# mako443/Text2Pos-CVPR2022

Measured on AMD Instinct MI355X. Metric: cells+queries encoded/sec and top-k retrieval QPS, 256-pt cells, 12k-cell DB, higher is better.
Workload: dtype f16x3 (fp32 operands split hi+lo into fp16, 3 f16 MFMAs, fp32 accumulate; fp32-class error) for the encoders / f64 MFMA for the ranking

## Files before the change

### text2pos-cvpr2022_amd/csrc/sa_rows.hip

```cpp
#ifndef T2P_RABL
#define T2P_RABL 0
#endif
#include "t2p_common.h"

namespace t2p {
namespace {

typedef __attribute__((address_space(3))) void lds_void;
typedef const __attribute__((address_space(1))) void gl_void;

__device__ __forceinline__ constexpr int rows_load_slot(int s, int c) {
    if (s == 0) return c == 0 || c == 4 ? -1 : 10 + (c < 4 ? c - 1 : c - 2);
    if (s == 1) return c == 1 ? 16 : (c == 3 ? 17 : -1);
    if (s == 4) return (c & 1) ? 18 + (c >> 1) : -1;
    if (s == 5) return (c & 1) ? 22 + (c >> 1) : -1;
    return -1;
}
#ifndef T2P_WA_HI_STEPS
#define T2P_WA_HI_STEPS 3
#endif
constexpr int WA_HI_STEPS = T2P_WA_HI_STEPS;
__device__ __forceinline__ constexpr bool w_in_agpr(bool lo_plane, int s) { return lo_plane || s < WA_HI_STEPS; }
__device__ __forceinline__ void mfma_w(f32x16& c, const half8& a, const half8& w, bool agpr, bool zero) {
    if (zero) {
        if (agpr) asm volatile("v_mfma_f32_32x32x16_f16 %0, %1, %2, 0" : "=a"(c) : "v"(a), "a"(w));
        else asm volatile("v_mfma_f32_32x32x16_f16 %0, %1, %2, 0" : "=a"(c) : "v"(a), "v"(w));
    } else {
        if (agpr) asm volatile("v_mfma_f32_32x32x16_f16 %0, %1, %2, %0" : "+a"(c) : "v"(a), "a"(w));
        else asm volatile("v_mfma_f32_32x32x16_f16 %0, %1, %2, %0" : "+a"(c) : "v"(a), "v"(w));
    }
}
#define SB() __builtin_amdgcn_sched_barrier(0)
#if T2P_RABL & 2
#define DS_MAX_STR "; no atomic %0 %1 %2"
#else
#define DS_MAX_STR "ds_max_f32 %0, %1 offset:%2"
#endif

constexpr int kSubR = 1024;

template <int K, int N, int NC, int NW>
struct RowsCfg {
    static constexpr int NT = 64 * NW;
    static constexpr int ND = 2 * NC;
    static constexpr int S16 = K / 16, NTW = N / 32;
    static constexpr int MAXR = NC * 33;
    static constexpr int ROWS_CHUNKS = (MAXR * 2 + 1023) / 1024;
    static constexpr int ROWS_BUF = ROWS_CHUNKS * 1024;
    static constexpr int BT_STRIDE = K * 4 + 16;
    static constexpr int CPOS_BUF = 3 * NC * 4;
    static constexpr int ACC_OFF = 0;
    static constexpr int XROW = kSaTailCode;
    static constexpr int BT_OFF = ACC_OFF + (NC + 1) * N * 4;
    static constexpr int ROWS_OFF = BT_OFF + NC * BT_STRIDE;
    static constexpr int CPOS_OFF = ROWS_OFF + 3 * ROWS_BUF;
    static constexpr int NR_OFF = CPOS_OFF + 2 * CPOS_BUF;
    static constexpr int SB_OFF = NR_OFF + kSubR * 2;
    static constexpr int DSTL_OFF = SB_OFF + kSubR * 4;
    static constexpr size_t lds_bytes() { return (size_t)(DSTL_OFF + NW * 64 + 1023) / 1024 * 1024; }
    static_assert(K % 32 == 0 && N % 32 == 0 && NC % 64 == 0 && (NC * N / 4) % NT == 0, "shape");
    static_assert(K == 128, "rows_load_slot schedules the loads of eight MFMA steps per tile");
    static_assert(XROW == NC && (NC & (NC - 1)) == 0 && XROW * N * 4 <= 0xFFFF && XROW < 128, "shared tail slot");
};

__device__ __forceinline__ void wait_all_vm() { asm volatile("s_waitcnt vmcnt(0)" ::: "memory"); }

struct TileRef {
    int gi, r0, n;
};

template <int K, int N, int NC, int NW>
__global__ __launch_bounds__(64 * NW, 1) void k_sa_rows(SaParams p) {
    using C = RowsCfg<K, N, NC, NW>;
    extern __shared__ __attribute__((aligned(16))) char lds[];
    int* acc_lds = (int*)(lds + C::ACC_OFF);
    uint16_t* nr = (uint16_t*)(lds + C::NR_OFF);
    int* sbase = (int*)(lds + C::SB_OFF);

    const int tid = threadIdx.x, lane = tid & 63;
    const int wave = __builtin_amdgcn_readfirstlane(tid >> 6);
    const int h = lane >> 5, rr = lane & 31;
    const uint32_t dstl_addr = (uint32_t)(C::DSTL_OFF + wave * 64);

    half8 w_hi[C::NTW][C::S16], w_lo[C::NTW][C::S16];
    {
        const uint4* wp = (const uint4*)p.W_x3;
        constexpr int PLANE_U4 = (N / 32) * C::S16 * 64;
#pragma unroll
        for (int nt = 0; nt < C::NTW; nt++)
#pragma unroll
            for (int s = 0; s < C::S16; s++) {
                const int kb = 16 * s + 8 * h;
                const int half_ = kb / (K / 2), step_ = (kb % (K / 2)) / 8;
                const int idx = (((nt * C::S16 + step_) * 2 + half_) * 32) + rr;
                w_hi[nt][s] = __builtin_bit_cast(half8, wp[idx]);
                w_lo[nt][s] = __builtin_bit_cast(half8, wp[PLANE_U4 + idx]);
                if (w_in_agpr(false, s)) asm volatile("" : "=a"(w_hi[nt][s]) : "0"(w_hi[nt][s]));
                asm volatile("" : "=a"(w_lo[nt][s]) : "0"(w_lo[nt][s]));
            }
    }
    f32x4 bias4;
    {
        const int c4 = tid % (N / 4);
        bias4 = *(const f32x4*)(p.bias + c4 * 4);
    }
    constexpr int QPR = K / 4;
    constexpr int CGS = C::NT / QPR;
    constexpr int CPT = NC / CGS;
    static_assert(C::NT % QPR == 0 && NC % CGS == 0, "centroid table build");
    const int cq = tid % QPR, cg = tid / QPR;
    const f32x4 wq0 = *(const f32x4*)(p.wp + cq * 4), wq1 = *(const f32x4*)(p.wp + K + cq * 4),
                wq2 = *(const f32x4*)(p.wp + 2 * K + cq * 4);

    for (int i = tid; i < (NC + 1) * N; i += C::NT) acc_lds[i] = (int)0xFF800000;
    int gtop = 0;

    const int g_begin = p.bounds_ws[blockIdx.x], g_end = p.bounds_ws[blockIdx.x + 1];

    auto dma16 = [&](const void* base, uint32_t voff, uint32_t lds_off) {
        __builtin_amdgcn_global_load_lds((gl_void*)((const char*)base + voff), (lds_void*)(lds + lds_off), 16, 0, 0);
    };
    auto dma_rows = [&](int g) {
        const char* src = (const char*)(p.rows + (int64_t)g * C::MAXR);
        const uint32_t dst = (uint32_t)(C::ROWS_OFF + (g % 3) * C::ROWS_BUF);
#pragma unroll
        for (int c = 0; c < C::ROWS_CHUNKS; c++) {
            if (c % NW != wave) continue;
            uint32_t off = (uint32_t)(c * 1024 + lane * 16);
            if (off + 16 > (uint32_t)(C::MAXR * 2)) off = 0;
            dma16(src, off, dst + c * 1024);
        }
    };
    auto dma_cpos = [&](int g) {
        if (wave != (NW > 1 ? 1 : 0)) return;
        const uint32_t dst = (uint32_t)(C::CPOS_OFF + (g & 1) * C::CPOS_BUF);
#pragma unroll
        for (int e = 0; e < 3; e++)
#pragma unroll
            for (int b = 0; b < NC / 64; b++) {
                const float* src = p.out + ((int64_t)g * NC + b * 64 + lane) * (int64_t)p.ldo + N + e;
                __builtin_amdgcn_global_load_lds((gl_void*)src, (lds_void*)(lds + dst + (e * NC + b * 64) * 4), 4, 0, 0);
            }
    };

    for (int ga = g_begin; ga < g_end; ga += kSubR) {
        const int cnt = (g_end - ga) < kSubR ? (g_end - ga) : kSubR;
        wait_all_vm();
        __syncthreads();
        for (int i = tid; i < cnt; i += C::NT) {
            const int g = ga + i;
            nr[i] = p.n_rows[g];
            const int first = p.first[g];
            sbase[i] = first * C::ND + (g - first) * NC;
        }
        dma_rows(ga);
        if (cnt > 1) dma_rows(ga + 1);
        dma_cpos(ga);
        wait_all_vm();
        __syncthreads();

        auto rows_of = [&](int gi) { return __builtin_amdgcn_readfirstlane((int)nr[gi]); };
        auto tile_meta = [&](int gi, int r0, int n) -> uint32_t {
            int idx = r0 + rr;
            idx = idx < n ? idx : n - 1;
            const uint16_t* rows_l = (const uint16_t*)(lds + C::ROWS_OFF + ((ga + gi) % 3) * C::ROWS_BUF);
            return (uint32_t)rows_l[idx];
        };
        auto row_byte = [&](int gi, uint32_t sb0, uint32_t m) -> uint32_t {
            const uint32_t src = m & 0xFFu, d = m >> 8;
            const uint32_t g = (uint32_t)(ga + gi);
            const uint32_t srow = (d & 0x80u) ? (sb0 + src) : (g * (uint32_t)C::ND + src);
            return srow * (uint32_t)(K * 4);
        };
        constexpr int AHEAD = 5;
        const uint32_t hoff = (uint32_t)(h * 32);
        auto load_half = [&](uint32_t roff, int s_, int j, f32x4 (&x)[2]) {
            if constexpr (!(T2P_RABL & 1)) x[j] = *(const f32x4*)((const char*)p.A + (size_t)roff + (size_t)(s_ * 64 + j * 16));
        };
        auto load_step = [&](uint32_t roff, int s_, f32x4 (&x)[2]) {
            load_half(roff, s_, 0, x);
            load_half(roff, s_, 1, x);
        };

        auto flush = [&](int g, int t0) {
            float* o = p.out + (int64_t)g * NC * (int64_t)p.ldo;
            int top = gtop;
            static_assert(C::NT % (N / 4) == 0, "a thread keeps its column quad over the drain");
            if (t0 < NC) {
                f32x4* const ax = (f32x4*)(acc_lds + C::XROW * N + (tid % (N / 4)) * 4);
                const f32x4 xq = *ax;
#pragma unroll 1
                for (int c = tid / (N / 4); c < NC; c += C::NT / (N / 4)) {
                    if (c < t0) continue;
                    f32x4* a = (f32x4*)(acc_lds + c * N + (tid % (N / 4)) * 4);
                    f32x4 r = *a;
#pragma unroll
                    for (int e = 0; e < 4; e++) r[e] = fmaxf(r[e], xq[e]);
                    *a = r;
                }
                lds_barrier();
                typedef int i32x4 __attribute__((ext_vector_type(4)));
                if (tid < N / 4) *(i32x4*)ax = i32x4{(int)0xFF800000, (int)0xFF800000, (int)0xFF800000, (int)0xFF800000};
            }
#pragma unroll
            for (int k = 0; k < NC * N / 4 / C::NT; k++) {
                const int i = tid + k * C::NT;
                const int c = i / (N / 4), c4 = i % (N / 4);
                typedef int i32x4 __attribute__((ext_vector_type(4)));
                f32x4* a = (f32x4*)(acc_lds + c * N + c4 * 4);
                const f32x4 raw = *a;
                f32x4 v;
#pragma unroll
                for (int e = 0; e < 4; e++) {
                    const float r = fmaxf(raw[e] + bias4[e], 0.f);
                    const int bits = __float_as_int(r);
                    top = bits > top ? bits : top;
                    v[e] = r * p.out_scale;
                }
                *(f32x4*)(o + c * (int64_t)p.ldo + c4 * 4) = v;
                *(i32x4*)a = i32x4{(int)0xFF800000, (int)0xFF800000, (int)0xFF800000, (int)0xFF800000};
            }
            gtop = top;
        };
        auto build_b = [&](int g) {
            const float* cp = (const float*)(lds + C::CPOS_OFF + (g & 1) * C::CPOS_BUF);
#pragma unroll
            for (int i = 0; i < CPT; i++) {
                const int c = cg + CGS * i;
                const float px = cp[c], py = cp[NC + c], pz = cp[2 * NC + c];
                f32x4 v;
#pragma unroll
                for (int e = 0; e < 4; e++) {
                    float a = px * wq0[e];
                    a = fmaf(py, wq1[e], a);
                    a = fmaf(pz, wq2[e], a);
                    v[e] = a;
                }
                *(f32x4*)(lds + C::BT_OFF + c * C::BT_STRIDE + cq * 16) = v;
            }
        };

        build_b(ga);
        if (cnt > 2) dma_rows(ga + 2);
        if (cnt > 1) dma_cpos(ga + 1);
        lds_barrier();

        bool cur_fetched = false;
        uint32_t m_cur = 0;
        uint32_t roff_cur = 0;
        f32x4 xw[C::S16][2];
#pragma unroll
        for (int s0 = 0; s0 < C::S16; s0++) xw[s0][0] = xw[s0][1] = f32x4{0.f, 0.f, 0.f, 0.f};

        for (int gi = 0; gi < cnt; gi++) {
            const int n_g = rows_of(gi), n_g1 = gi + 1 < cnt ? rows_of(gi + 1) : 0;
            const uint32_t sb_g = (uint32_t)__builtin_amdgcn_readfirstlane(sbase[gi]);
            const uint32_t sb_g1 = gi + 1 < cnt ? (uint32_t)__builtin_amdgcn_readfirstlane(sbase[gi + 1]) : 0u;
            int t0;
            {
                static_assert(NC == 64, "one lane per centroid");
                const uint32_t* cp = (const uint32_t*)(lds + C::CPOS_OFF + ((ga + gi) & 1) * C::CPOS_BUF);
                const bool same = lane > 0 && cp[lane] == cp[0] && cp[NC + lane] == cp[NC] && cp[2 * NC + lane] == cp[2 * NC];
                const unsigned long long tm = __ballot(same);
                t0 = tm ? (int)__builtin_ctzll(tm) : NC;
            }
            int r0 = wave * 32;
            bool have = r0 < n_g;
            const bool did_tile = have;
            half8 a_hi, a_lo;
            f32x16 acc[C::NTW];
            bool pend = false;
            uint2 fourp[4] = {};
            auto read_step = [&](int s, uint32_t brow_, f32x4 (&x)[2], f32x4 (&b)[2]) {
#pragma unroll
                for (int j = 0; j < 2; j++) {
                    x[j] = xw[s][j];
                    b[j] = *(const f32x4*)(lds + brow_ + s * 64 + j * 16);
                }
            };
            auto prep_a = [&](int pr, const f32x4 (&x)[2], const f32x4 (&b)[2], float (&v)[2]) {
                const int j = pr >> 1, e0 = (pr & 1) * 2;
                v[0] = fmaxf(x[j][e0] - b[j][e0], 0.f);
                v[1] = fmaxf(x[j][e0 + 1] - b[j][e0 + 1], 0.f);
            };
            auto prep_b = [&](const float (&v)[2], uint32_t& wh, uint32_t& wl) {
                const fp16x2 hh = cvt_pk_f16(v[0], v[1]);
                wh = __builtin_bit_cast(uint32_t, hh);
                wl = split_lo_pk(hh, v[0], v[1]);
            };
            typedef uint32_t u32x4 __attribute__((ext_vector_type(4)));
            auto row_addr = [&](const uint2 (&f4)[4], int e) -> uint32_t {
                const uint32_t pair = (e & 2) ? f4[e >> 2].y : f4[e >> 2].x;
                return (uint32_t)(C::ACC_OFF + rr * 4) + ((e & 1) ? (pair >> 16) : (pair & 0xFFFFu));
            };

            if (have) {
                if (!cur_fetched) {
                    m_cur = tile_meta(gi, r0, n_g);
                    roff_cur = row_byte(gi, sb_g, m_cur) + hoff;
#pragma unroll
                    for (int s0 = 0; s0 < AHEAD; s0++) load_step(roff_cur, s0, xw[s0]);
                }
                {
                    f32x4 x[2], b[2];
                    read_step(0, (uint32_t)C::BT_OFF + ((m_cur >> 8) & (uint32_t)(NC - 1)) * (uint32_t)C::BT_STRIDE + (uint32_t)(h * 32), x, b);
                    uint32_t nh[4], nl[4];
#pragma unroll
                    for (int pr = 0; pr < 4; pr++) {
                        float v[2];
                        prep_a(pr, x, b, v);
                        prep_b(v, nh[pr], nl[pr]);
                    }
                    a_hi = __builtin_bit_cast(half8, u32x4{nh[0], nh[1], nh[2], nh[3]});
                    a_lo = __builtin_bit_cast(half8, u32x4{nl[0], nl[1], nl[2], nl[3]});
                }
            }
            while (have) {
                const bool chain = r0 + NW * 32 < n_g;
                const bool nxt_ok = chain || (gi + 1 < cnt && wave * 32 < n_g1);
                const int gi_n = chain ? gi : (nxt_ok ? gi + 1 : gi);
                const int r0_n = chain ? r0 + NW * 32 : (nxt_ok ? wave * 32 : r0);
                const int n_n = (chain || !nxt_ok) ? n_g : n_g1;
                const uint32_t sb_n = (chain || !nxt_ok) ? sb_g : sb_g1;
                uint32_t m_nxt = tile_meta(gi_n, r0_n, n_n);
                uint32_t roff_n = roff_cur;
                const uint32_t dl = (m_cur >> 8) & 127u;
                const uint32_t brow = (uint32_t)C::BT_OFF + (dl & (uint32_t)(NC - 1)) * (uint32_t)C::BT_STRIDE + (uint32_t)(h * 32);
                asm volatile("ds_write_b16 %0, %1" ::"v"(dstl_addr + (uint32_t)(rr * 2)), "v"(dl * (uint32_t)(N * 4)) : "memory");
                uint2 four[4];

                uint32_t brow_n = 0;

#pragma unroll
                for (int s = 0; s < C::S16 - 1; s++) {
                    f32x4 x[2], b[2];
                    read_step(s + 1, brow, x, b);
                    if (s == C::S16 - 2) {
                        const uint32_t a4 = dstl_addr + (uint32_t)(h * 8);
                        asm volatile("ds_read_b64 %0, %4\n\tds_read_b64 %1, %4 offset:16\n\tds_read_b64 %2, %4 offset:32\n\t"
                                     "ds_read_b64 %3, %4 offset:48"
                                     : "=&v"(four[0]), "=&v"(four[1]), "=&v"(four[2]), "=&v"(four[3]) : "v"(a4) : "memory");
                    }
                    SB();
                    if (s == 0) {
#pragma unroll
                        for (int nt = 0; nt < C::NTW - 1; nt++) mfma_w(acc[nt], a_hi, w_hi[nt][0], w_in_agpr(false, 0), true);
                        if (pend) {
#pragma unroll
                            for (int e = 0; e < 16; e++)
                                asm volatile(DS_MAX_STR ::"v"(row_addr(fourp, e)), "a"(acc[C::NTW - 1][e]), "n"((C::NTW - 1) * 128) : "memory");
                        }
                        mfma_w(acc[C::NTW - 1], a_hi, w_hi[C::NTW - 1][0], w_in_agpr(false, 0), true);
                    } else {
#pragma unroll
                        for (int nt = 0; nt < C::NTW; nt++) mfma_w(acc[nt], a_hi, w_hi[nt][s], w_in_agpr(false, s), false);
                    }
                    SB();
                    uint32_t nh[4], nl[4];
                    float v[2];
                    uint32_t rowbyte_n = 0;
#pragma unroll
                    for (int c = 0; c < 8; c++) {
                        if ((c & 1) == 0) prep_a(c >> 1, x, b, v);
                        else prep_b(v, nh[c >> 1], nl[c >> 1]);
                        if (s == 0) {
                            if (c == 2) rowbyte_n = row_byte(gi_n, sb_n, m_nxt);
                            if (c == 4) roff_n = rowbyte_n + hoff;
                            if (c == 6) brow_n = (uint32_t)C::BT_OFF + ((m_nxt >> 8) & (uint32_t)(NC - 1)) * (uint32_t)C::BT_STRIDE + (uint32_t)(h * 32);
                        }
                        {
                            const int ld = rows_load_slot(s, c);
                            if (ld >= 0) load_half(ld < 2 * C::S16 ? roff_cur : roff_n, (ld >> 1) % C::S16, ld & 1, xw[(ld >> 1) % C::S16]);
                        }
                        if (c < 4) mfma_w(acc[c], a_hi, w_lo[c][s], w_in_agpr(true, s), false);
                        else mfma_w(acc[c - 4], a_lo, w_hi[c - 4][s], w_in_agpr(false, s), false);
                        SB();
                    }
                    a_hi = __builtin_bit_cast(half8, u32x4{nh[0], nh[1], nh[2], nh[3]});
                    a_lo = __builtin_bit_cast(half8, u32x4{nl[0], nl[1], nl[2], nl[3]});
                }
                {
                    constexpr int s = C::S16 - 1;
                    f32x4 x[2], b[2];
                    if (chain) read_step(0, brow_n, x, b);
                    asm volatile("s_waitcnt lgkmcnt(0)\n\ts_nop 1" : "+v"(four[0]), "+v"(four[1]), "+v"(four[2]), "+v"(four[3])::"memory");
                    SB();
                    uint32_t ad[16];
                    uint32_t nh[4], nl[4];
                    float v[2];
#pragma unroll
                    for (int i = 0; i < 3 * C::NTW; i++) {
                        const int nt = i / 3, k = i % 3;
                        if (k == 0) mfma_w(acc[nt], a_hi, w_hi[nt][s], w_in_agpr(false, s), false);
                        else if (k == 1) mfma_w(acc[nt], a_hi, w_lo[nt][s], w_in_agpr(true, s), false);
                        else mfma_w(acc[nt], a_lo, w_hi[nt][s], w_in_agpr(false, s), false);
                        if (i < 4) {
#pragma unroll
                            for (int e = 4 * i; e < 4 * i + 4; e++) ad[e] = row_addr(four, e);
                        }
                        if (chain && i < 8) {
                            if ((i & 1) == 0) prep_a(i >> 1, x, b, v);
                            else prep_b(v, nh[i >> 1], nl[i >> 1]);
                        }
                        if (i >= 4 && ((i - 4) % 3) < 2 && (i - 4) / 3 < C::NTW - 1) {
                            const int nb = (i - 4) / 3, e0 = ((i - 4) % 3) * 8;
#pragma unroll
                            for (int e = e0; e < e0 + 8; e++)
                                asm volatile(DS_MAX_STR ::"v"(ad[e]), "a"(acc[nb][e]), "n"(nb * 128) : "memory");
                        }
                        SB();
                    }
                    if (chain) {
                        a_hi = __builtin_bit_cast(half8, u32x4{nh[0], nh[1], nh[2], nh[3]});
                        a_lo = __builtin_bit_cast(half8, u32x4{nl[0], nl[1], nl[2], nl[3]});
#pragma unroll
                        for (int q = 0; q < 4; q++) fourp[q] = four[q];
                        pend = true;
                    } else {
                        asm volatile("s_nop 15\n\ts_nop 15" ::: "memory");
#pragma unroll
                        for (int e = 0; e < 16; e++)
                            asm volatile(DS_MAX_STR ::"v"(ad[e]), "a"(acc[C::NTW - 1][e]), "n"((C::NTW - 1) * 128) : "memory");
                        pend = false;
                    }
                }
                have = chain;
                r0 = r0_n;
                cur_fetched = nxt_ok;
                m_cur = m_nxt;
                roff_cur = roff_n;
            }
            if (!did_tile) cur_fetched = false;
            if (!did_tile) wait_all_vm();
            if constexpr (!(T2P_RABL & 16)) lds_barrier();
            if constexpr (!(T2P_RABL & 4)) flush(ga + gi, t0);
            if (gi + 1 < cnt) {
                if constexpr (!(T2P_RABL & 4)) build_b(ga + gi + 1);
                if (gi + 3 < cnt) dma_rows(ga + gi + 3);
                if (gi + 2 < cnt) dma_cpos(ga + gi + 2);
            }
            if constexpr (!(T2P_RABL & 16)) lds_barrier();
        }
    }
    wait_all_vm();
    uint32_t gbits = 0;
    guard_track_bits(gbits, gtop);
    if (p.amax_out != nullptr && lane == 0 && gbits != 0u)
        atomicMax(p.amax_out, __float_as_uint(__uint_as_float(gbits) * p.out_scale));
}

}

bool sa_rows_selected(int H, int Cout, const SaParams& p) {
    return H == 128 && Cout == 128 && p.W_x3 != nullptr && p.wp != nullptr;
}

int sa_rows_launch_shape(int64_t n_obj, int* tile_rows, int* n_wg) {
    int n = matrix_wgs();
    if (n > 1024) n = 1024;
    if (n > n_obj) n = (int)n_obj;
    *tile_rows = 4 * 32;
    *n_wg = n;
    return 0;
}

int launch_sa_rows(int H, int Cout, const SaParams& p, hipStream_t st) {
    if (!(H == 128 && Cout == 128 && p.n_cent == 64 && p.n_dense == 128 && p.wp && p.W_x3)) {
        set_error("sa_rows: built for SA level 2 (H = C = 128, 64 centroids of 128 points, f16x3, LDS centroid table)");
        return T2P_E_UNSUPPORTED;
    }
    using C = RowsCfg<128, 128, 64, 4>;
    auto kern = k_sa_rows<128, 128, 64, 4>;
    T2P_TRY(reserve_lds((const void*)kern, C::lds_bytes(), "sa_rows"));
    if (p.n_obj <= 0) return 0;
    T2P_CHECK_ARG(p.n_obj < (1 << 30) && p.n_obj * p.n_dense * (int64_t)H * 4 < 0xffffffffLL,
                  "sa_rows: chunk too large for 32-bit table offsets");
    T2P_CHECK_ARG((((uintptr_t)p.A | (uintptr_t)p.rows | (uintptr_t)p.out | (uintptr_t)p.W_x3) & 15) == 0 && p.ldo % 4 == 0,
                  "sa_rows: tables must be 16-byte aligned");
    int tr, n_wg;
    sa_rows_launch_shape(p.n_obj, &tr, &n_wg);
    if (!p.balanced) T2P_TRY(launch_sa_balance(p, tr, n_wg, st));
    ProfScope ps_("ws_edge_sa_k128_n128", st);
    T2P_REPEAT(ps_) hipLaunchKernelGGL(kern, dim3(n_wg), dim3(C::NT), C::lds_bytes(), st, p);
    T2P_CHECK_LAUNCH("sa_rows");
    return 0;
}

}
```

Before: 161,000.

## Double-buffer accumulator and centroid tables to drop the per-group trailing barrier

Double-buffers the LDS accumulator and centroid-bias tables by group parity and triple-buffers the centroid positions. This removes the second barrier after each group's flush and lets waves drain and rebuild rows without a block-wide sync. The drain and the build of the table two groups ahead are split per wave, shifted toward waves that finish their tiles early. The tail-row fold is merged into the drain and the work is unrolled in fours. The cost is more LDS use and extra prologue work, plus fragile load-balancing arithmetic that carries a risk of races.

```diff
diff --git a/text2pos-cvpr2022_amd/csrc/sa_rows.hip b/text2pos-cvpr2022_amd/csrc/sa_rows.hip
--- a/text2pos-cvpr2022_amd/csrc/sa_rows.hip
+++ b/text2pos-cvpr2022_amd/csrc/sa_rows.hip
@@ -49,15 +49,20 @@
     static constexpr int ROWS_BUF = ROWS_CHUNKS * 1024;
     static constexpr int BT_STRIDE = K * 4 + 16;
     static constexpr int CPOS_BUF = 3 * NC * 4;
+    static constexpr int XROW = kSaTailCode;
+    static constexpr int ACC_BUF = (NC + 1) * N * 4;
+    static constexpr int BT_BUF = NC * BT_STRIDE;
+    static constexpr int UNITS = NC / 2;
     static constexpr int ACC_OFF = 0;
-    static constexpr int XROW = kSaTailCode;
-    static constexpr int BT_OFF = ACC_OFF + (NC + 1) * N * 4;
-    static constexpr int ROWS_OFF = BT_OFF + NC * BT_STRIDE;
+    static constexpr int BT_OFF = ACC_OFF + 2 * ACC_BUF;
+    static constexpr int ROWS_OFF = BT_OFF + 2 * BT_BUF;
     static constexpr int CPOS_OFF = ROWS_OFF + 3 * ROWS_BUF;
-    static constexpr int NR_OFF = CPOS_OFF + 2 * CPOS_BUF;
+    static constexpr int NR_OFF = CPOS_OFF + 3 * CPOS_BUF;
     static constexpr int SB_OFF = NR_OFF + kSubR * 2;
     static constexpr int DSTL_OFF = SB_OFF + kSubR * 4;
     static constexpr size_t lds_bytes() { return (size_t)(DSTL_OFF + NW * 64 + 1023) / 1024 * 1024; }
+    static_assert(DSTL_OFF + NW * 64 <= 160 * 1024, "LDS budget of a gfx950 CU");
+    static_assert(N / 4 == 32 && (NW == 2 || NW == 4), "a half wave drains one row; the drain shares are worked out for two or four waves");
     static_assert(K % 32 == 0 && N % 32 == 0 && NC % 64 == 0 && (NC * N / 4) % NT == 0, "shape");
     static_assert(K == 128, "rows_load_slot schedules the loads of eight MFMA steps per tile");
     static_assert(XROW == NC && (NC & (NC - 1)) == 0 && XROW * N * 4 <= 0xFFFF && XROW < 128, "shared tail slot");
@@ -105,14 +110,12 @@
         bias4 = *(const f32x4*)(p.bias + c4 * 4);
     }
     constexpr int QPR = K / 4;
-    constexpr int CGS = C::NT / QPR;
-    constexpr int CPT = NC / CGS;
-    static_assert(C::NT % QPR == 0 && NC % CGS == 0, "centroid table build");
-    const int cq = tid % QPR, cg = tid / QPR;
+    static_assert(QPR == 32, "centroid table build: a half wave writes one table row");
+    const int cq = tid % QPR;
     const f32x4 wq0 = *(const f32x4*)(p.wp + cq * 4), wq1 = *(const f32x4*)(p.wp + K + cq * 4),
                 wq2 = *(const f32x4*)(p.wp + 2 * K + cq * 4);
 
-    for (int i = tid; i < (NC + 1) * N; i += C::NT) acc_lds[i] = (int)0xFF800000;
+    for (int i = tid; i < 2 * (NC + 1) * N; i += C::NT) acc_lds[i] = (int)0xFF800000;
     int gtop = 0;
 
     const int g_begin = p.bounds_ws[blockIdx.x], g_end = p.bounds_ws[blockIdx.x + 1];
@@ -133,7 +136,7 @@
     };
     auto dma_cpos = [&](int g) {
         if (wave != (NW > 1 ? 1 : 0)) return;
-        const uint32_t dst = (uint32_t)(C::CPOS_OFF + (g & 1) * C::CPOS_BUF);
+        const uint32_t dst = (uint32_t)(C::CPOS_OFF + (g % 3) * C::CPOS_BUF);
 #pragma unroll
         for (int e = 0; e < 3; e++)
 #pragma unroll
@@ -156,6 +159,7 @@
         dma_rows(ga);
         if (cnt > 1) dma_rows(ga + 1);
         dma_cpos(ga);
+        if (cnt > 1) dma_cpos(ga + 1);
         wait_all_vm();
         __syncthreads();
 
@@ -182,67 +186,88 @@
             load_half(roff, s_, 1, x);
         };
 
-        auto flush = [&](int g, int t0) {
-            float* o = p.out + (int64_t)g * NC * (int64_t)p.ldo;
+        constexpr int SHARE_UNROLL = 4;
+        auto drain_rows = [&](int g, int t0, int u0, int u1, bool tail) {
+            typedef int i32x4 __attribute__((ext_vector_type(4)));
+            const i32x4 ninf = i32x4{(int)0xFF800000, (int)0xFF800000, (int)0xFF800000, (int)0xFF800000};
+            int* const acc = (int*)(lds + C::ACC_OFF + (g & 1) * C::ACC_BUF);
+            float* const o = p.out + (int64_t)g * NC * (int64_t)p.ldo + rr * 4;
             int top = gtop;
-            static_assert(C::NT % (N / 4) == 0, "a thread keeps its column quad over the drain");
-            if (t0 < NC) {
-                f32x4* const ax = (f32x4*)(acc_lds + C::XROW * N + (tid % (N / 4)) * 4);
-                const f32x4 xq = *ax;
+            f32x4* const ax = (f32x4*)(acc + C::XROW * N + rr * 4);
+            f32x4 xq = f32x4{0.f, 0.f, 0.f, 0.f};
+            if (tail) xq = *ax;
 #pragma unroll 1
-                for (int c = tid / (N / 4); c < NC; c += C::NT / (N / 4)) {
-                    if (c < t0) continue;
-                    f32x4* a = (f32x4*)(acc_lds + c * N + (tid % (N / 4)) * 4);
-                    f32x4 r = *a;
-#pragma unroll
-                    for (int e = 0; e < 4; e++) r[e] = fmaxf(r[e], xq[e]);
-                    *a = r;
-                }
-                lds_barrier();
-                typedef int i32x4 __attribute__((ext_vector_type(4)));
-                if (tid < N / 4) *(i32x4*)ax = i32x4{(int)0xFF800000, (int)0xFF800000, (int)0xFF800000, (int)0xFF800000};
-            }
-#pragma unroll
-            for (int k = 0; k < NC * N / 4 / C::NT; k++) {
-                const int i = tid + k * C::NT;
-                const int c = i / (N / 4), c4 = i % (N / 4);
-                typedef int i32x4 __attribute__((ext_vector_type(4)));
-                f32x4* a = (f32x4*)(acc_lds + c * N + c4 * 4);
-                const f32x4 raw = *a;
-                f32x4 v;
-#pragma unroll
-                for (int e = 0; e < 4; e++) {
-                    const float r = fmaxf(raw[e] + bias4[e], 0.f);
-                    const int bits = __float_as_int(r);
-                    top = bits > top ? bits : top;
-                    v[e] = r * p.out_scale;
-                }
-                *(f32x4*)(o + c * (int64_t)p.ldo + c4 * 4) = v;
-                *(i32x4*)a = i32x4{(int)0xFF800000, (int)0xFF800000, (int)0xFF800000, (int)0xFF800000};
-            }
+            for (int u = u0; u < u1; u += SHARE_UNROLL) {
+                f32x4* a[SHARE_UNROLL];
+                f32x4 raw[SHARE_UNROLL];
+                int c[SHARE_UNROLL];
+#pragma unroll
+                for (int k = 0; k < SHARE_UNROLL; k++) {
+                    const int uk = u + k < u1 ? u + k : u1 - 1;
+                    c[k] = 2 * uk + h;
+                    a[k] = (f32x4*)(acc + c[k] * N + rr * 4);
+                    raw[k] = *a[k];
+                }
+#pragma unroll
+                for (int k = 0; k < SHARE_UNROLL; k++) *(i32x4*)a[k] = ninf;
+#pragma unroll
+                for (int k = 0; k < SHARE_UNROLL; k++) {
+                    if (tail) {
+                        const bool fold = c[k] >= t0;
+#pragma unroll
+                        for (int e = 0; e < 4; e++) {
+                            const float m = fmaxf(raw[k][e], xq[e]);
+                            raw[k][e] = fold ? m : raw[k][e];
+                        }
+                    }
+                    f32x4 v;
+#pragma unroll
+                    for (int e = 0; e < 4; e++) {
+                        const float r = fmaxf(raw[k][e] + bias4[e], 0.f);
+                        const int bits = __float_as_int(r);
+                        top = bits > top ? bits : top;
+                        v[e] = r * p.out_scale;
+                    }
+                    *(f32x4*)(o + c[k] * (int64_t)p.ldo) = v;
+                }
+            }
+            if (tail && lane < N / 4) *(i32x4*)ax = ninf;
             gtop = top;
         };
-        auto build_b = [&](int g) {
-            const float* cp = (const float*)(lds + C::CPOS_OFF + (g & 1) * C::CPOS_BUF);
-#pragma unroll
-            for (int i = 0; i < CPT; i++) {
-                const int c = cg + CGS * i;
-                const float px = cp[c], py = cp[NC + c], pz = cp[2 * NC + c];
-                f32x4 v;
-#pragma unroll
-                for (int e = 0; e < 4; e++) {
-                    float a = px * wq0[e];
-                    a = fmaf(py, wq1[e], a);
-                    a = fmaf(pz, wq2[e], a);
-                    v[e] = a;
-                }
-                *(f32x4*)(lds + C::BT_OFF + c * C::BT_STRIDE + cq * 16) = v;
+        auto build_rows = [&](int g, int u0, int u1) {
+            const float* cp = (const float*)(lds + C::CPOS_OFF + (g % 3) * C::CPOS_BUF);
+            char* const bt = lds + C::BT_OFF + (g & 1) * C::BT_BUF + rr * 16;
+#pragma unroll 1
+            for (int u = u0; u < u1; u += SHARE_UNROLL) {
+                int c[SHARE_UNROLL];
+                float px[SHARE_UNROLL], py[SHARE_UNROLL], pz[SHARE_UNROLL];
+#pragma unroll
+                for (int k = 0; k < SHARE_UNROLL; k++) {
+                    const int uk = u + k < u1 ? u + k : u1 - 1;
+                    c[k] = 2 * uk + h;
+                    px[k] = cp[c[k]], py[k] = cp[NC + c[k]], pz[k] = cp[2 * NC + c[k]];
+                }
+#pragma unroll
+                for (int k = 0; k < SHARE_UNROLL; k++) {
+                    f32x4 v;
+#pragma unroll
+                    for (int e = 0; e < 4; e++) {
+                        float a = px[k] * wq0[e];
+                        a = fmaf(py[k], wq1[e], a);
+                        a = fmaf(pz[k], wq2[e], a);
+                        v[e] = a;
+                    }
+                    *(f32x4*)(bt + c[k] * C::BT_STRIDE) = v;
+                }
             }
         };
 
-        build_b(ga);
-        if (cnt > 2) dma_rows(ga + 2);
-        if (cnt > 1) dma_cpos(ga + 1);
+        build_rows(ga, wave * C::UNITS / NW, (wave + 1) * C::UNITS / NW);
+        if (cnt > 1) build_rows(ga + 1, wave * C::UNITS / NW, (wave + 1) * C::UNITS / NW);
+        if (cnt > 2) {
+            dma_rows(ga + 2);
+            dma_cpos(ga + 2);
+        }
         lds_barrier();
 
         bool cur_fetched = false;
@@ -259,11 +284,14 @@
             int t0;
             {
                 static_assert(NC == 64, "one lane per centroid");
-                const uint32_t* cp = (const uint32_t*)(lds + C::CPOS_OFF + ((ga + gi) & 1) * C::CPOS_BUF);
+                const uint32_t* cp = (const uint32_t*)(lds + C::CPOS_OFF + ((ga + gi) % 3) * C::CPOS_BUF);
                 const bool same = lane > 0 && cp[lane] == cp[0] && cp[NC + lane] == cp[NC] && cp[2 * NC + lane] == cp[2 * NC];
                 const unsigned long long tm = __ballot(same);
                 t0 = tm ? (int)__builtin_ctzll(tm) : NC;
             }
+            const uint32_t par = (uint32_t)((ga + gi) & 1);
+            const uint32_t acc_rr = (uint32_t)C::ACC_OFF + par * (uint32_t)C::ACC_BUF + (uint32_t)(rr * 4);
+            const uint32_t bt_h = (uint32_t)C::BT_OFF + par * (uint32_t)C::BT_BUF + (uint32_t)(h * 32);
             int r0 = wave * 32;
             bool have = r0 < n_g;
             const bool did_tile = have;
@@ -291,7 +319,7 @@
             typedef uint32_t u32x4 __attribute__((ext_vector_type(4)));
             auto row_addr = [&](const uint2 (&f4)[4], int e) -> uint32_t {
                 const uint32_t pair = (e & 2) ? f4[e >> 2].y : f4[e >> 2].x;
-                return (uint32_t)(C::ACC_OFF + rr * 4) + ((e & 1) ? (pair >> 16) : (pair & 0xFFFFu));
+                return acc_rr + ((e & 1) ? (pair >> 16) : (pair & 0xFFFFu));
             };
 
             if (have) {
@@ -303,7 +331,7 @@
                 }
                 {
                     f32x4 x[2], b[2];
-                    read_step(0, (uint32_t)C::BT_OFF + ((m_cur >> 8) & (uint32_t)(NC - 1)) * (uint32_t)C::BT_STRIDE + (uint32_t)(h * 32), x, b);
+                    read_step(0, bt_h + ((m_cur >> 8) & (uint32_t)(NC - 1)) * (uint32_t)C::BT_STRIDE, x, b);
                     uint32_t nh[4], nl[4];
 #pragma unroll
                     for (int pr = 0; pr < 4; pr++) {
@@ -325,7 +353,7 @@
                 uint32_t m_nxt = tile_meta(gi_n, r0_n, n_n);
                 uint32_t roff_n = roff_cur;
                 const uint32_t dl = (m_cur >> 8) & 127u;
-                const uint32_t brow = (uint32_t)C::BT_OFF + (dl & (uint32_t)(NC - 1)) * (uint32_t)C::BT_STRIDE + (uint32_t)(h * 32);
+                const uint32_t brow = bt_h + (dl & (uint32_t)(NC - 1)) * (uint32_t)C::BT_STRIDE;
                 asm volatile("ds_write_b16 %0, %1" ::"v"(dstl_addr + (uint32_t)(rr * 2)), "v"(dl * (uint32_t)(N * 4)) : "memory");
                 uint2 four[4];
 
@@ -366,7 +394,7 @@
                         if (s == 0) {
                             if (c == 2) rowbyte_n = row_byte(gi_n, sb_n, m_nxt);
                             if (c == 4) roff_n = rowbyte_n + hoff;
-                            if (c == 6) brow_n = (uint32_t)C::BT_OFF + ((m_nxt >> 8) & (uint32_t)(NC - 1)) * (uint32_t)C::BT_STRIDE + (uint32_t)(h * 32);
+                            if (c == 6) brow_n = bt_h + ((m_nxt >> 8) & (uint32_t)(NC - 1)) * (uint32_t)C::BT_STRIDE;
                         }
                         {
                             const int ld = rows_load_slot(s, c);
@@ -433,13 +461,35 @@
             if (!did_tile) cur_fetched = false;
             if (!did_tile) wait_all_vm();
             if constexpr (!(T2P_RABL & 16)) lds_barrier();
-            if constexpr (!(T2P_RABL & 4)) flush(ga + gi, t0);
-            if (gi + 1 < cnt) {
-                if constexpr (!(T2P_RABL & 4)) build_b(ga + gi + 1);
-                if (gi + 3 < cnt) dma_rows(ga + gi + 3);
-                if (gi + 2 < cnt) dma_cpos(ga + gi + 2);
-            }
-            if constexpr (!(T2P_RABL & 16)) lds_barrier();
+            {
+                const int g = ga + gi;
+                const int rem = ((n_g1 + 31) >> 5) & (NW - 1);
+                const int nl = NW - rem;
+                auto div_small = [](int x, int d) { return d == 1 ? x : (d == 2 ? x >> 1 : (x * 171) >> 9); };
+                const int ut = t0 >> 1;
+                int u0 = 0, u1 = 0;
+                if (nl == 1) {
+                    if (wave == NW - 1) u1 = C::UNITS;
+                } else {
+                    int ulast = nl == 2 ? C::UNITS / 2 : (nl == 3 ? C::UNITS * 2 / 3 : C::UNITS * 3 / 4);
+                    ulast = ut < ulast ? ut : ulast;
+                    if (wave == NW - 1) {
+                        u0 = ulast;
+                        u1 = C::UNITS;
+                    } else if (wave >= rem) {
+                        u0 = div_small(ulast * (wave - rem), nl - 1);
+                        u1 = div_small(ulast * (wave - rem + 1), nl - 1);
+                    }
+                }
+                if constexpr (!(T2P_RABL & 4)) {
+                    drain_rows(g, t0, u0, u1, wave == NW - 1 && t0 < NC);
+                    if (gi + 2 < cnt) build_rows(g + 2, u0, u1);
+                }
+                if (gi + 3 < cnt) {
+                    dma_rows(g + 3);
+                    dma_cpos(g + 3);
+                }
+            }
         }
     }
     wait_all_vm();
```

Result: no change. 161,000, median of 2 (-0.0%).
